# yinwoods/k8s-scheduler

Measured on AMD Instinct MI355X. Metric: pod-node evaluations/sec, higher is better.
Workload: dtype f64

## Files before the change

### include/ksched.h

```cpp
#ifndef KSCHED_H
#define KSCHED_H

#include <stddef.h>
#include <stdint.h>

#ifdef __cplusplus
extern "C" {
#endif

#define KSCHED_ABI_VERSION 6

#define KSCHED_OK 0
#define KSCHED_E_INVALID (-1)
#define KSCHED_E_DEVICE (-2)
#define KSCHED_E_PARSE (-3)
#define KSCHED_E_STATE (-4)
#define KSCHED_E_NOMEM (-5)
#define KSCHED_E_UNKNOWN_NODE (-6)

#define KSCHED_NO_FIT (-1)
#define KSCHED_NO_POSITIVE_SCORE (-2)
#define KSCHED_GANG_REJECTED (-3)

#define KSCHED_MODE_EXACT 0
// ... 158 lines not shown

int ksched_upload_pods(ksched_ctx *ctx, int64_t p, const int64_t *req_cpu, const int64_t *req_mem,
                       const int64_t *req_pods, const uint64_t *selector);
int ksched_run(ksched_ctx *ctx);
int ksched_set_timeout(ksched_ctx *ctx, int32_t persist_ms);
int ksched_sync(ksched_ctx *ctx);
int ksched_download_results(ksched_ctx *ctx, int64_t p, int32_t *out_idx, double *out_score, int32_t *out_feasible);
int ksched_get_stats(const ksched_ctx *ctx, ksched_stats *out);
int ksched_get_commit_stamps(const ksched_ctx *ctx, int32_t n, int64_t *out);
int ksched_get_seed_stats(const ksched_ctx *ctx, int64_t *out);
int ksched_set_timing(ksched_ctx *ctx, int32_t timing, int32_t every);

int ksched_selftest_fastdiv(ksched_ctx *ctx, int64_t n, const double *a, const double *b, double *out_native,
                            double *out_fast);
int ksched_selftest_score(ksched_ctx *ctx, int64_t n, const int64_t *req, const int64_t *alloc, double *out_score,
                          double *out_upper, double *out_recip, int32_t *out_flags);
int ksched_selftest_price_key(ksched_ctx *ctx, int64_t n, const float *price, double *out_key);
int ksched_selftest_screen(ksched_ctx *ctx, int64_t n, const int64_t *req, const int64_t *alloc, float *out_f32,
                           uint32_t *out_u32);
int ksched_selftest_rec_w(ksched_ctx *ctx, int64_t n, const float *w, const float *w2, uint32_t *out);
int ksched_selftest_threshold(ksched_ctx *ctx, int64_t n, const float *L, const uint32_t *rec, int32_t *out);
int ksched_selftest_seed(ksched_ctx *ctx, int64_t n, const float *v, const float *L, const uint32_t *flags,
                         const uint32_t *x, uint32_t *out);
int ksched_selftest_wave(ksched_ctx *ctx, int64_t ncases, const uint64_t *sort_code, const int32_t *sort_idx,
                         const double *key, const int32_t *idx, const int32_t *aux, const int32_t *cut,
                         const int32_t *nv, uint64_t *out_u64, int32_t *out_i32);
int ksched_selftest_list(ksched_ctx *ctx, int64_t n, int32_t steps, const double *key, const int32_t *idx,
                         double *out_key, int32_t *out_idx);
int ksched_selftest_slots(ksched_ctx *ctx, int64_t n, int32_t steps, const uint32_t *x, uint32_t *out);
int ksched_selftest_rank_merge(ksched_ctx *ctx, int32_t K, int32_t R, int32_t nb, const void *blocks, void *out_rec,
                               int64_t *out_fc);
int ksched_selftest_commit(ksched_ctx *ctx, int32_t impl, int32_t K, int32_t B, int32_t priority, int32_t domain,
                           int32_t use_labels, int32_t fast53, int32_t nb, const int64_t *rc, const int64_t *rm,
                           const int64_t *rp, const uint64_t *sel, const void *lists, const int64_t *fc0,
                           const void *xin, int32_t *out_idx, double *out_score, int32_t *out_feas, void *out_x,
                           int64_t *out_ctl);

int ksched_parse_cpu(const char *s, int64_t *out);
int ksched_parse_memory(const char *s, int64_t *out);
int ksched_parse_pods(const char *s, int64_t *out);
int ksched_parse_price(const char *s, float *out);

int ksched_pack_nodes(int64_t n, const char *const *names, const char *const *cap_cpu,
                      const char *const *cap_mem, const char *const *cap_pods,
                      int64_t nb, const char *const *bound_node, const int64_t *cont_off,
                      const char *const *cont_cpu, const char *const *cont_mem,
// ... 9 lines not shown
```

### k8s-scheduler_amd/csrc/ksched_commit.h

```cpp
#pragma once

#include <hip/hip_runtime.h>

#include <type_traits>

#ifndef KSCHED_XCHG_DEBUG
#define KSCHED_XCHG_DEBUG 0
#endif

#include "ksched_pipe.h"

namespace ksched {

namespace {

constexpr int kSpcHashBits = 11;
constexpr int kSpcHash = 1 << kSpcHashBits;
template <bool LAG3>
constexpr int spc_slots() { return LAG3 ? 192 : 128; }
static_assert(spc_slots<true>() + 1 <= kRescueMaxT, "RescueReq::ti must hold the persistent commit's touched slots");
constexpr int kSpcInvalid = kSpcHash - 1;
constexpr int kGS = 14;

constexpr uint64_t kSkipKeyBits = 0x7ff8000000000badull;
__device__ __forceinline__ double skip_key() { return __longlong_as_double((long long)kSkipKeyBits); }
__device__ __forceinline__ float screen_y(int64_t a, double y) {
    return (a > 0 && a < (1ll << 52)) ? (float)y : __builtin_nanf("");
}

struct alignas(8) SpcSlot {
    int32_t idx;
    int32_t mine;
    int64_t sb[3];
    int64_t cur[3];
    uint64_t labels;
    float price;
    int32_t pad;
};
static_assert(sizeof(SpcSlot) == 72, "SpcSlot");

struct SpcSmem {
    int32_t *hk;
    int64_t *s0;
    double *iy;
    int32_t *HP;
    uint32_t *tkc;
    int32_t *ti;
    SpcSlot *T;
    double *S;
    double *LK;
    int32_t *LI;
    int8_t *D;
    int32_t *fcg;
    int32_t *dfacc;
    int32_t *gn;
    int32_t *gq;
    int32_t *gs;
    double *pbk;
    int64_t *pbx;
    int32_t *ctl;
    int32_t *own;
    uint64_t *GS;
    float *thr;
    int16_t *x2s;
    float *rb2;
};

// ... 271 lines not shown
        m.pbk = reinterpret_cast<double *>(p); p += (size_t)kSpcWaves * 64 * sizeof(double);
        m.pbx = reinterpret_cast<int64_t *>(p); p += (size_t)kSpcWaves * 64 * sizeof(int64_t);
        m.LK = reinterpret_cast<double *>(p); p += (size_t)K * 64 * sizeof(double);
        m.GS = reinterpret_cast<uint64_t *>(p); p += 64 * kGS * sizeof(uint64_t);
        m.D = reinterpret_cast<int8_t *>(p); p += 64 * 64;
        m.T = reinterpret_cast<SpcSlot *>(p); p += (size_t)spc_slots<LAG3>() * sizeof(SpcSlot);
        m.LI = reinterpret_cast<int32_t *>(p); p += (size_t)K * 64 * sizeof(int32_t);
        m.HP = reinterpret_cast<int32_t *>(p); p += (size_t)K * 64 * sizeof(int32_t);
        m.hk = reinterpret_cast<int32_t *>(p); p += kSpcHash * sizeof(int32_t);
        m.tkc = reinterpret_cast<uint32_t *>(p); p += 64 * sizeof(uint32_t);
        m.ti = reinterpret_cast<int32_t *>(p); p += spc_slots<LAG3>() * sizeof(int32_t);
        m.fcg = reinterpret_cast<int32_t *>(p); p += 64 * sizeof(int32_t);
        m.dfacc = reinterpret_cast<int32_t *>(p); p += 64 * sizeof(int32_t);
        m.gn = reinterpret_cast<int32_t *>(p); p += 64 * sizeof(int32_t);
        m.gq = reinterpret_cast<int32_t *>(p); p += 64 * sizeof(int32_t);
        m.gs = reinterpret_cast<int32_t *>(p); p += 64 * sizeof(int32_t);
        m.ctl = reinterpret_cast<int32_t *>(p); p += 4 * sizeof(int32_t);
        m.thr = reinterpret_cast<float *>(p); p += 64 * sizeof(float);
        m.x2s = reinterpret_cast<int16_t *>(p); p += 64 * sizeof(int16_t);
        m.S = reinterpret_cast<double *>(p);
        m.own = reinterpret_cast<int32_t *>(m.pbk);
        m.s0 = reinterpret_cast<int64_t *>(m.D);
        m.iy = reinterpret_cast<double *>(m.GS);
        m.rb2 = reinterpret_cast<float *>(m.dfacc);
    }
    const int nb = (int)((A.pods.p - p0 < A.B) ? A.pods.p - p0 : A.B);
    const bool pj = lane < nb;
    const LanePods lp = pre ? *pre : load_lane_pods<LAB>(A.pods, p0, nb);
    const int64_t rc = lp.rc, rm = lp.rm, rp = lp.rp;
    const uint64_t sel = lp.sel;
    constexpr int kHeadPer = (64 * K + kSpcThreads - 1) / kSpcThreads;
    uint64_t w0[kHeadPer], w1[kHeadPer];
    int64_t fc0v = 0;
    int cut0 = 0;
    int32_t thr0 = 0;
    auto load_lists = [&]() {
        fc0v = (wave == 0 && pj) ? load_i64<COH>(A.fc0 + lane) : 0;
        cut0 = (wave == 0 && pj) ? (int32_t)(uint32_t)(load_i64<COH>(
                                       reinterpret_cast<const int64_t *>(A.lists + (size_t)lane * K) + 6) >> 32) : 0;
        if (SCR)
            thr0 = (wave == 0 && pj) ? (int32_t)(uint32_t)(load_i64<COH>(
                                           reinterpret_cast<const int64_t *>(A.lists + (size_t)lane * K + 1) + 6) >> 32) : 0;
#pragma unroll
        for (int u = 0; u < kHeadPer; ++u) {
            const int e = tid + u * kSpcThreads;
            w0[u] = 0; w1[u] = 0;
            if (e < 64 * K && e / K < nb) {
                const uint64_t *w = reinterpret_cast<const uint64_t *>(A.lists + e);
                if (COH) { w0[u] = ld_coh(w); w1[u] = ld_coh(w + 1); }
                else { w0[u] = w[0]; w1[u] = w[1]; }
            }
        }
    };
    if constexpr (!COH) load_lists();

    int n1 = 0, n2 = 0, nin = 0;
    uint64_t dbg_x1 = 0;
    (void)dbg_x1;
    const double rcf = (double)rc, rmf = (double)rm, rpf = (double)rp;
    const double y3 = recip(3.0);
    double *Srow = m.S + (size_t)lane * kSpcRow;
    uint64_t smv[3] = {0, 0, 0};
    auto key_inherited = [&](int ne, auto sl) {
        int dfl = 0;
        double pk = -__builtin_inf();
        int32_t pi = kNoIdx, ps = -1;
        const float thrf = SCR ? m.thr[lane] : 0.0f;
        const float qc = screen_req(rc), qm = screen_req(rm), qp = screen_req(rp);
        int64_t nex = 0;
        for (int e = wave; e < ne; e += kSpcWaves) {
            const int t = sl(e);
            const SpcSlot &x = m.T[t];
            const int64_t *x0 = m.s0 + e * 3;
            const bool f0 = fits(rc, rm, rp, sel, x0[0], x0[1], x0[2], x.labels, LAB);
            const bool f1 = fits(rc, rm, rp, sel, x.cur[0], x.cur[1], x.cur[2], x.labels, LAB);
            dfl += (int)f1 - (int)f0;
            const double *yy = m.iy + e * 6;
            bool need = true;
            if constexpr (SCR) {
                bool lo;
                const float v = screen_pair(qc, qm, qp, screen_y(x.cur[0], yy[3]), screen_y(x.cur[1], yy[4]),
                                            screen_y(x.cur[2], yy[5]), x.cur[0] >= rc, x.cur[1] >= rm, x.cur[2] >= rp, &lo);
                need = pj && !(v < thrf);
            }
            double k;
            if (!SCR || __ballot(need) != 0) {
                ++nex;
                const bool el = pair_key_fast<PRIO, DOM, F53>(f1, rc, rm, rp, rcf, rmf, rpf, x.cur[0], x.cur[1], x.cur[2],
                                                              yy[0], yy[1], yy[2], yy[3], yy[4], yy[5], y3, x.price, &k);
                k = el ? k : -__builtin_inf();
            } else {
                k = skip_key();
            }
            Srow[t] = k;
            const bool up = k != -__builtin_inf() && better(k, x.idx, pk, pi);
            pk = up ? k : pk; pi = up ? x.idx : pi; ps = up ? t : ps;
        }
        m.pbk[wave * 64 + lane] = pk;
        m.pbx[wave * 64 + lane] = ((int64_t)ps << 32) | (uint32_t)pi;
        if (dfl != 0) atomicAdd(&m.dfacc[lane], dfl);
        if (SCR && A.dbg && lane == 0 && wave < ne) {
            atomicAdd(reinterpret_cast<unsigned long long *>(&A.dbg[16]), (unsigned long long)((ne - 1 - wave) / kSpcWaves + 1));
            atomicAdd(reinterpret_cast<unsigned long long *>(&A.dbg[17]), (unsigned long long)nex);
        }
    };
    auto hash_lists = [&]() {
#pragma unroll
        for (int u = 0; u < kHeadPer; ++u) {
            const int e = tid + u * kSpcThreads;
            if (e < 64 * K) {
                const int j = e / K, q = e % K;
                const bool v = (uint32_t)(w1[u] >> 32) != 0;
                const double key = v ? __longlong_as_double((long long)w0[u]) : -__builtin_inf();
                const int32_t idx = v ? (int32_t)(uint32_t)w1[u] : kNoIdx;
                m.LK[q * 64 + j] = key;
                m.LI[q * 64 + j] = idx;
                m.HP[q * 64 + j] = idx == kNoIdx ? kSpcInvalid : spc_pos_insert(m.hk, idx);
// ... 132 lines not shown
        if (A.xp && A.xp->xdbg && wave == 0) {
            int64_t x = lane < n1 ? (int64_t)dbg_mix((uint64_t)xi.idx ^ ((uint64_t)xi.cur[0] << 20), (uint64_t)xi.cur[1] ^
                                                     (uint64_t)xi.cur[2] ^ (uint64_t)xi.sb[0], lane) : 0;
            x = wave_sum_i64(x);
            dbg_x1 = (uint64_t)x;
        }
#endif
        if (wave == 0) {
            int h = 0;
            bool dup = false;
            if (lane < n1) {
                h = spc_pos_insert(m.hk, xi.idx);
                dup = (m.tkc[h >> 5] >> (h & 31)) & 1u;
            }
            const uint64_t nm = __ballot(lane < n1 && !dup);
            const int slot = dup ? m.own[h] : n2 + __popcll(nm & ((1ull << lane) - 1ull));
            if (lane < n1) {
                SpcSlot &x = m.T[slot];
                x.idx = xi.idx; x.mine = 0;
                for (int r = 0; r < 3; ++r) { m.s0[lane * 3 + r] = xi.sb[r]; x.sb[r] = xi.cur[r]; x.cur[r] = xi.cur[r]; }
                x.labels = xi.labels; x.price = xi.price; x.pad = 0;
                m.ti[slot] = xi.idx;
                m.gs[lane] = slot;
                stage_state(m.iy + lane * 6, xi.cur);
                if (dup) m.x2s[slot] = -1;
                else atomicOr(&m.tkc[h >> 5], 1u << (h & 31));
            }
            if (lane == 0) m.ctl[3] = n2 + __popcll(nm);
        }
        __syncthreads();
        if (tid == 0 && A.trace_row) A.trace_row[23] = wall_clock64();
        nin = m.ctl[3];
        key_inherited(n1, [&](int e) { return (int)m.gs[e]; });
        __syncthreads();
        if (tid == 0 && A.trace_row) A.trace_row[24] = wall_clock64();
    }

    int32_t fcc = 0;
    double rbk = -__builtin_inf();
    int32_t rbi = kNoIdx, rbs = -1;
    constexpr bool RB2 = COH && PRIO == kPrioResource && DOM == kDomAll;
    bool trk = false;
    int cv = 0, cut = 0;
    int32_t my_idx = 0, my_feas = 0;
    int32_t my_src = 0;
    double my_score = 0.0;
    int32_t my_g = -2, my_q = -1, my_s = -1, my_h = kSpcInvalid;
// ... 158 lines not shown
            const bool in = lane >= c && lane < cend;
            if (in && my_g == 0) my_g = m.LI[my_q * 64 + lane];
            m.gn[lane] = in ? my_g : -2;
            m.gq[lane] = my_q;
            m.gs[lane] = my_s;
            m.fcg[lane] = 0;
            if (lane == 0) { m.ctl[0] = c; m.ctl[1] = cend; }
        }
        __syncthreads();
        if (first && tr1) tr1[49] = wall_clock64();
        if (dbg) { const uint64_t t = __builtin_amdgcn_s_memtime(); t_s1 += t - t_mark; t_mark = t; }
        const int rc0 = m.ctl[0], rce = m.ctl[1];
        {
            double pk = -__builtin_inf();
            int32_t pi = kNoIdx, ps = -1;
            if (wave == 0 && lane >= rc0 && lane < rce && m.gn[lane] >= 0) {
                const uint64_t *src = reinterpret_cast<const uint64_t *>(A.lists + (size_t)lane * K + m.gq[lane]) + 2;
                uint64_t v[5];
#pragma unroll
                for (int w = 0; w < 5; ++w) v[w] = COH ? ld_coh(src + w) : src[w];
                const int64_t n0 = wsub((int64_t)v[0], rc), n1 = wsub((int64_t)v[1], rm), n2 = wsub((int64_t)v[2], 1);
                const double nf0 = (double)n0, nf1 = (double)n1, nf2 = (double)n2;
                uint64_t *o = m.GS + (size_t)lane * kGS;
#pragma unroll
                for (int w = 0; w < 5; ++w) o[w] = v[w];
                o[5] = (uint64_t)n0; o[6] = (uint64_t)n1; o[7] = (uint64_t)n2;
                o[8] = (uint64_t)__double_as_longlong(nf0); o[9] = (uint64_t)__double_as_longlong(nf1);
                o[10] = (uint64_t)__double_as_longlong(nf2);
                o[11] = (uint64_t)__double_as_longlong(recip_or_zero(n0, nf0));
                o[12] = (uint64_t)__double_as_longlong(recip_or_zero(n1, nf1));
                o[13] = (uint64_t)__double_as_longlong(recip_or_zero(n2, nf2));
            }
            __syncthreads();
            const float thrf = SCR ? m.thr[lane] : 0.0f;
            const float qc = screen_req(rc), qm = screen_req(rm), qp = screen_req(rp);
            int64_t nev = 0, nex = 0;
            for (int k = rc0 + wave; k < rce; k += kSpcWaves) {
                const int32_t g = __builtin_amdgcn_readfirstlane(m.gn[k]);
                if (g < 0) continue;
                const int s = __builtin_amdgcn_readfirstlane(m.gs[k]);
                const uint64_t *gsk = m.GS + (size_t)k * kGS;
                const int64_t a0 = (int64_t)gsk[0], a1 = (int64_t)gsk[1], a2 = (int64_t)gsk[2];
                const uint64_t lab = gsk[3];
                const float pr = __uint_as_float((uint32_t)gsk[4]);
                const int64_t n0 = (int64_t)gsk[5], n1 = (int64_t)gsk[6], n2 = (int64_t)gsk[7];
                const bool fo = fits(rc, rm, rp, sel, a0, a1, a2, lab, LAB);
                const bool fn = fits(rc, rm, rp, sel, n0, n1, n2, lab, LAB);
                const int d = (int)fn - (int)fo;
                const double ny0 = __longlong_as_double((long long)gsk[11]), ny1 = __longlong_as_double((long long)gsk[12]),
                             ny2 = __longlong_as_double((long long)gsk[13]);
                bool need = true;
                if constexpr (SCR) {
                    bool lo;
                    const float v = screen_pair(qc, qm, qp, screen_y(n0, ny0), screen_y(n1, ny1), screen_y(n2, ny2),
                                                n0 >= rc, n1 >= rm, n2 >= rp, &lo);
                    need = lane > k && pj && !(v < thrf);
                }
                double kv;
                ++nev;
                if (!SCR || __ballot(need) != 0) {
                    ++nex;
                    const bool el = pair_key_fast<PRIO, DOM, F53>(
                        fn, rc, rm, rp, rcf, rmf, rpf, n0, n1, n2, __longlong_as_double((long long)gsk[8]),
                        __longlong_as_double((long long)gsk[9]), __longlong_as_double((long long)gsk[10]), ny0, ny1, ny2,
                        y3, pr, &kv);
                    kv = el ? kv : -__builtin_inf();
                } else {
                    kv = skip_key();
                }
                Srow[s] = kv;
                m.D[k * 64 + lane] = (int8_t)d;
                if (lane > k) {
                    if (d != 0) atomicAdd(&m.fcg[lane], d);
                    const bool up = kv != -__builtin_inf() && better(kv, g, pk, pi);
                    pk = up ? kv : pk; pi = up ? g : pi; ps = up ? s : ps;
                }
                if (lane == 0) {
                    SpcSlot &x = m.T[s];
                    x.idx = g; x.mine = 1;
                    x.sb[0] = a0; x.sb[1] = a1; x.sb[2] = a2;
                    x.cur[0] = n0; x.cur[1] = n1; x.cur[2] = n2;
                    x.labels = lab; x.price = pr; x.pad = 0;
                    m.ti[s] = g;
                }
            }
            m.pbk[wave * 64 + lane] = pk;
            m.pbx[wave * 64 + lane] = ((int64_t)ps << 32) | (uint32_t)pi;
            if (SCR && A.dbg && lane == 0 && nev) {
                atomicAdd(reinterpret_cast<unsigned long long *>(&A.dbg[18]), (unsigned long long)nev);
                atomicAdd(reinterpret_cast<unsigned long long *>(&A.dbg[19]), (unsigned long long)nex);
            }
        }
        __syncthreads();
        if (first && tr1) tr1[50] = wall_clock64();
        if (dbg) { const uint64_t t = __builtin_amdgcn_s_memtime(); t_s2 += t - t_mark; t_mark = t; }
        if (wave == 0) {
            ++nrounds;
            const int cend = rce;
            double tk = rbk;
            int32_t ti = rbi, ts = rbs;
            for (int w = 0; w < kSpcWaves; ++w) {
                const double k = m.pbk[w * 64 + lane];
                const int64_t x = m.pbx[w * 64 + lane];
                const int32_t xi = (int32_t)(uint32_t)x;
                const bool up = k != -__builtin_inf() && better(k, xi, tk, ti);
                tk = up ? k : tk; ti = up ? xi : ti; ts = up ? (int32_t)(x >> 32) : ts;
// ... 145 lines not shown
                    if (kf != 0) {
                        ++placed;
                        int64_t b0, b1, b2;
                        uint64_t lab;
                        float pr;
                        if (kf == 1 && rescued) {
                            b0 = ro.a[0]; b1 = ro.a[1]; b2 = ro.a[2]; lab = ro.labels; pr = ro.price;
                            s = nT++;
                        } else if (kf == 1) {
                            int64_t ra[3];
                            load_rec_state<COH>(A.lists + (size_t)f * K + qf, ra, &lab, &pr);
                            b0 = ra[0]; b1 = ra[1]; b2 = ra[2];
                            s = nT++;
                        } else {
                            const SpcSlot &x = m.T[s];
                            b0 = x.cur[0]; b1 = x.cur[1]; b2 = x.cur[2]; lab = x.labels; pr = x.price;
                        }
                        const int64_t n0 = wsub(b0, rl64(rc, f)), n1 = wsub(b1, rl64(rm, f)), n2 = wsub(b2, 1);
                        const bool fo = fits(rc, rm, rp, sel, b0, b1, b2, lab, LAB);
                        const bool fn = fits(rc, rm, rp, sel, n0, n1, n2, lab, LAB);
                        fcc += (int32_t)fn - (int32_t)fo;
                        double kv;
                        if constexpr (SCR) {
                            const double nf0 = (double)n0, nf1 = (double)n1, nf2 = (double)n2;
                            const double ny0 = recip_or_zero(n0, nf0), ny1 = recip_or_zero(n1, nf1),
                                         ny2 = recip_or_zero(n2, nf2);
                            bool lo;
                            const float v = screen_pair(screen_req(rc), screen_req(rm), screen_req(rp), screen_y(n0, ny0),
                                                        screen_y(n1, ny1), screen_y(n2, ny2), n0 >= rc, n1 >= rm, n2 >= rp,
                                                        &lo);
                            const bool need = lane > f && pj && !(v < m.thr[lane]);
                            const bool any = __ballot(need) != 0;
                            if (any) {
                                const bool el = pair_key_fast<PRIO, DOM, F53>(fn, rc, rm, rp, rcf, rmf, rpf, n0, n1, n2, nf0,
                                                                              nf1, nf2, ny0, ny1, ny2, y3, pr, &kv);
                                kv = el ? kv : -__builtin_inf();
                            } else {
                                kv = skip_key();
                            }
                            if (A.dbg && lane == 0) {
                                atomicAdd(reinterpret_cast<unsigned long long *>(&A.dbg[20]), 1ull);
                                if (any) atomicAdd(reinterpret_cast<unsigned long long *>(&A.dbg[21]), 1ull);
                            }
                        } else {
                            kv = lane_key<PRIO, DOM, LAB, F53>(fn, rc, rm, rp, rcf, rmf, rpf, n0, n1, n2, y3, pr);
                        }
                        Srow[s] = kv;
                        if (lane == 0) {
                            SpcSlot &x = m.T[s];
                            if (kf == 1) {
                                x.idx = wi;
                                x.sb[0] = b0; x.sb[1] = b1; x.sb[2] = b2;
                                x.labels = lab; x.price = pr; x.pad = 0;
                                m.ti[s] = wi;
                                const int pos = rescued ? spc_pos_insert(m.hk, wi) : m.HP[qf * 64 + f];
                                m.tkc[pos >> 5] |= 1u << (pos & 31);
                            }
                            x.mine = 1;
                            x.cur[0] = n0; x.cur[1] = n1; x.cur[2] = n2;
                        }
                        lds_order();
                        const bool up = kv != -__builtin_inf() && better(kv, wi, rbk, rbi);
// ... 161 lines not shown
            if (done < nb) __hip_atomic_fetch_add(st + 1, 1ull, __ATOMIC_RELAXED, __HIP_MEMORY_SCOPE_AGENT);
            __hip_atomic_fetch_add(st + 2, (unsigned long long)placed, __ATOMIC_RELAXED, __HIP_MEMORY_SCOPE_AGENT);
            if (nresc) __hip_atomic_fetch_add(st + 4, (unsigned long long)nresc, __ATOMIC_RELAXED, __HIP_MEMORY_SCOPE_AGENT);
        }
        if (threadIdx.x == 0) A.loc->rescue_credit = rcredit - 4 * nresc;
    }
    return 1;
}

template <int K, int NT = kSpcThreads, bool LAG3 = false>
constexpr size_t spc_small_bytes() {
    return (size_t)(NT / 64) * 64 * 16 + (size_t)K * 64 * 8 + 64 * kGS * 8 + 64 * 64 + spc_slots<LAG3>() * sizeof(SpcSlot) +
           (size_t)K * 64 * 8 + (size_t)kSpcHash * 4 + 64 * 4 + spc_slots<LAG3>() * 4 + 5 * 64 * 4 + 16 + 64 * 4 + 64 * 2;
}
template <int K, int NT = kSpcThreads, bool LAG3 = false>
constexpr size_t spc_lds_bytes() {
    return (size_t)64 * (spc_slots<LAG3>() + 1) * 8 + (size_t)(NT / 64) * 64 * 16 + (size_t)K * 64 * 12 +
           spc_slots<LAG3>() * sizeof(SpcSlot) + (size_t)kSpcHash * 4 + (size_t)K * 64 * 4 + 64 * 4 +
           spc_slots<LAG3>() * 4 + 5 * 64 * 4 + 16 + 64 * kGS * 8 + 64 * 4 + 64 * 2 + 64 * 64;
}
static_assert(spc_lds_bytes<16>() <= 160 * 1024, "k_commit_spc LDS");
static_assert(spc_lds_bytes<16, kPipeThreads, true>() == spc_small_bytes<16, kPipeThreads, true>() + 64 * 193 * 8,
              "SpcSmem: S last");
static_assert(64 * 64 >= 128 * 3 * 8 && 64 * kGS * 8 >= 128 * 6 * 8, "SpcSmem prologue aliases");
static_assert((size_t)(kSpcThreads / 64) * 64 * 16 >= kSpcHash * 4 && (kPipeThreads / 64) * 64 * 16 >= kSpcHash * 4,
              "SpcSmem::own aliases pbk/pbx");

}
```

### k8s-scheduler_amd/csrc/ksched_data.hip

```cpp
#include <cmath>
#include <cstring>

#include <new>

#include "ksched_ctx.h"
#include "ksched_preempt.h"
#include "ksched_rank.h"

using namespace ksched;

static uint64_t uabs(int64_t v) { return v < 0 ? (uint64_t)0 - (uint64_t)v : (uint64_t)v; }

bool ksched::build_bound_table(int64_t n, int64_t nb, const int32_t *node_idx, const int64_t *cpu, const int64_t *mem,
                               const int32_t *prio, BoundTableHost *out, const char **why) {
    const int64_t blocks = (n + 63) / 64;
    out->seg.assign((size_t)n, 0);
    for (int64_t t = 0; t < nb; ++t) {
        if (node_idx[t] < 0 || node_idx[t] >= n) { *why = "node index out of range"; return false; }
        if (++out->seg[(size_t)node_idx[t]] > kBoundMaxPerNode) { *why = "more than KSCHED_BOUND_MAX_PER_NODE pods on one node"; return false; }
    }
    std::vector<int64_t> start((size_t)n + 1, 0);
    for (int64_t j = 0; j < n; ++j) start[(size_t)j + 1] = start[(size_t)j] + out->seg[(size_t)j];
    std::vector<int32_t> order((size_t)nb);
    {
// ... 375 lines not shown

int ksched_selftest_threshold(ksched_ctx *c, int64_t n, const float *L, const uint32_t *rec, int32_t *out) {
    if (!c || n < 0 || (n > 0 && (!L || !rec || !out))) return KSCHED_E_INVALID;
    if (n == 0) return KSCHED_OK;
    const size_t q = (size_t)n;
    return selftest_run(c, "selftest_threshold", {{L, nullptr, q * 4}, {rec, nullptr, q * 4}, {nullptr, out, q * 16}},
                        [&](const std::vector<void *> &p) {
                            return launch_selftest_threshold(n, (const float *)p[0], (const uint32_t *)p[1],
                                                             (int32_t *)p[2], c->stream);
                        });
}

int ksched_selftest_seed(ksched_ctx *c, int64_t n, const float *v, const float *L, const uint32_t *flags,
                         const uint32_t *x, uint32_t *out) {
    if (!c || n < 0 || (n > 0 && (!v || !L || !flags || !x || !out))) return KSCHED_E_INVALID;
    if (n == 0) return KSCHED_OK;
    const size_t q = (size_t)n;
    return selftest_run(c, "selftest_seed",
                        {{v, nullptr, q * 4}, {L, nullptr, q * 4}, {flags, nullptr, q * 4}, {x, nullptr, q * 24},
                         {nullptr, out, q * 20}},
                        [&](const std::vector<void *> &p) {
                            return launch_selftest_seed(n, (const float *)p[0], (const float *)p[1], (const uint32_t *)p[2],
                                                        (const uint32_t *)p[3], (uint32_t *)p[4], c->stream);
                        });
}

int ksched_selftest_wave(ksched_ctx *c, int64_t ncases, const uint64_t *sort_code, const int32_t *sort_idx,
                         const double *key, const int32_t *idx, const int32_t *aux, const int32_t *cut,
                         const int32_t *nv, uint64_t *out_u64, int32_t *out_i32) {
    if (!c || ncases < 0 || ncases > (1 << 20) ||
        (ncases > 0 && (!sort_code || !sort_idx || !key || !idx || !aux || !cut || !nv || !out_u64 || !out_i32)))
        return KSCHED_E_INVALID;
    if (ncases == 0) return KSCHED_OK;
    const size_t l = (size_t)ncases * 64;
    return selftest_run(c, "selftest_wave",
                        {{sort_code, nullptr, l * 6 * 8}, {sort_idx, nullptr, l * 6 * 4}, {key, nullptr, l * 8},
                         {idx, nullptr, l * 4}, {aux, nullptr, l * 4}, {cut, nullptr, (size_t)ncases * 4},
                         {nv, nullptr, (size_t)ncases * 4}, {nullptr, out_u64, l * 12 * 8}, {nullptr, out_i32, l * 13 * 4}},
                        [&](const std::vector<void *> &p) {
                            WaveTestArgs a{};
                            a.ncases = ncases;
                            a.scode = (const uint64_t *)p[0]; a.sidx = (const int32_t *)p[1];
                            a.key = (const double *)p[2]; a.kidx = (const int32_t *)p[3]; a.aux = (const int32_t *)p[4];
                            a.cut = (const int32_t *)p[5]; a.nv = (const int32_t *)p[6];
                            uint64_t *u = (uint64_t *)p[7];
                            int32_t *v = (int32_t *)p[8];
// ... 302 lines not shown
```

### k8s-scheduler_amd/csrc/ksched_kernels.h

```cpp
#pragma once

#include "ksched_device.h"

namespace ksched {

struct alignas(16) XRec {
    int32_t idx;
    int32_t pad;
    int64_t cur[3];
    int64_t sb[3];
    uint64_t labels;
    float price;
    int32_t pad2;
    int64_t pad3;
};
static_assert(sizeof(XRec) == 80, "XRec layout");

template <bool COH>
__device__ __forceinline__ void add_i64(int64_t *p, int64_t v) {
    if (COH) st_coh(p, (uint64_t)((int64_t)ld_coh(p) + v)); else *p += v;
}

struct alignas(16) XBuf {
    int32_t count;
// ... 165 lines not shown
    const int32_t *kidx, *aux;
    const int32_t *cut, *nv;
    uint64_t *ocode;
    int32_t *oidx;
    int32_t *rank;
    uint64_t *red_max;
    int64_t *red_sum;
    int32_t *red_min;
    uint64_t *red_or;
    uint64_t *ab_key;
    int32_t *ab_idx, *ab_aux;
    uint64_t *kcode;
    int32_t *thr;
};
hipError_t launch_selftest_score(int64_t n, const int64_t *req, const int64_t *alloc, double *score, double *upper,
                                 double *rcp, int32_t *flags, hipStream_t s);
hipError_t launch_selftest_price(int64_t n, const float *price, double *key, hipStream_t s);
hipError_t launch_selftest_screen(int64_t n, const int64_t *req, const int64_t *alloc, float *f, uint32_t *u,
                                  hipStream_t s);
hipError_t launch_selftest_rec_w(int64_t n, const float *w, const float *w2, uint32_t *out, hipStream_t s);
hipError_t launch_selftest_threshold(int64_t n, const float *L, const uint32_t *rec, int32_t *out, hipStream_t s);
hipError_t launch_selftest_seed(int64_t n, const float *v, const float *L, const uint32_t *flags, const uint32_t *x,
                                uint32_t *out, hipStream_t s);
hipError_t launch_selftest_wave(const WaveTestArgs &a, hipStream_t s);
hipError_t launch_selftest_list(int64_t n, int S, const double *key, const int32_t *idx, double *okey, int32_t *oidx,
                                hipStream_t s);
hipError_t launch_selftest_slots(int64_t n, int steps, const uint32_t *x, uint32_t *out, hipStream_t s);

#define KSCHED_DISPATCH(prio, dom, lab, f53, CALL)                                              \
    do {                                                                                        \
        if ((prio) == kPrioPrice) {                                                             \
            constexpr int P_ = kPrioPrice, D_ = kDomFeasible; constexpr bool F_ = false;        \
            if (lab) { constexpr bool L_ = true; return CALL; }                                 \
            else { constexpr bool L_ = false; return CALL; }                                    \
        }                                                                                       \
        constexpr int P_ = kPrioResource;                                                       \
        if ((dom) == kDomFeasible) {                                                            \
            constexpr int D_ = kDomFeasible;                                                    \
            if (lab) { constexpr bool L_ = true;                                                \
                if (f53) { constexpr bool F_ = true; return CALL; } else { constexpr bool F_ = false; return CALL; } } \
            else { constexpr bool L_ = false;                                                   \
                if (f53) { constexpr bool F_ = true; return CALL; } else { constexpr bool F_ = false; return CALL; } } \
        } else {                                                                                \
            constexpr int D_ = kDomAll;                                                         \
            if (lab) { constexpr bool L_ = true;                                                \
                if (f53) { constexpr bool F_ = true; return CALL; } else { constexpr bool F_ = false; return CALL; } } \
// ... 7 lines not shown
```

### k8s-scheduler_amd/csrc/ksched_selftest.hip

```cpp
#include <hip/hip_runtime.h>

#include <cstring>

#include "ksched_commit.h"
#include "ksched_ctx.h"
#include "ksched_merge.h"
#include "ksched_stream.h"

namespace ksched {

namespace {

struct PairOps {
    int64_t r[3], a[3];
    double rf[3], af[3], y[3], y3;
};
__device__ __forceinline__ PairOps load_ops(int64_t n, int64_t i, const int64_t *req, const int64_t *alloc) {
    PairOps o;
#pragma unroll
    for (int k = 0; k < 3; ++k) {
        o.r[k] = req[k * n + i];
        o.a[k] = alloc[k * n + i];
        o.rf[k] = (double)o.r[k];
        o.af[k] = (double)o.a[k];
// ... 92 lines not shown
    out[2 * n + i] = pk & 0xffffu;
    out[3 * n + i] = pk >> 16;
}

__global__ void k_selftest_threshold(int64_t n, const float *L, const uint32_t *rec, int32_t *out) {
    const int64_t i = (int64_t)blockIdx.x * blockDim.x + threadIdx.x;
    if (i >= n) return;
    const int tq = screen_rec_threshold(L[i]), tqn = screen_rec_threshold_nf(L[i]);
    out[i] = tq;
    out[n + i] = tqn;
    out[2 * n + i] = screen_rec_needed(rec[i], tq, tqn) ? 1 : 0;
    out[3 * n + i] = screen_rec_needed(rec[i], -1, -1) ? 1 : 0;
}

__global__ void k_selftest_seed(int64_t n, const float *v, const float *L, const uint32_t *flags, const uint32_t *x,
                                uint32_t *out) {
    const int64_t i = (int64_t)blockIdx.x * blockDim.x + threadIdx.x;
    if (i >= n) return;
    out[i] = screen_need(v[i], (flags[i] & 1u) != 0, (flags[i] & 2u) != 0, L[i]) ? 1u : 0u;
    uint32_t t[4] = {0u, 0u, 0u, 0u};
    for (int s = 0; s < 6; ++s) bound_insert<4>(t, x[s * n + i]);
#pragma unroll
    for (int q = 0; q < 4; ++q) out[(1 + q) * n + i] = t[q];
}

template <int RUN>
__device__ __forceinline__ void sort_case(const WaveTestArgs &A, int r, int64_t nl, int64_t i, int lane) {
    uint64_t c = A.scode[r * nl + i];
    int32_t x = A.sidx[r * nl + i];
    wave_sort_desc<RUN>(c, x, lane);
    A.ocode[r * nl + i] = c;
    A.oidx[r * nl + i] = x;
}

__global__ __launch_bounds__(64) void k_selftest_wave(WaveTestArgs A) {
    const int64_t cs = blockIdx.x;
    if (cs >= A.ncases || threadIdx.x >= 64) return;
    const int lane = (int)threadIdx.x;
    const int64_t nl = A.ncases * 64, i = cs * 64 + lane;
    sort_case<1>(A, 0, nl, i, lane);
    sort_case<2>(A, 1, nl, i, lane);
    sort_case<4>(A, 2, nl, i, lane);
    sort_case<8>(A, 3, nl, i, lane);
    sort_case<16>(A, 4, nl, i, lane);
    sort_case<32>(A, 5, nl, i, lane);
    const uint64_t c0 = A.scode[i];
// ... 79 lines not shown
}

namespace {
dim3 grid_of(int64_t n) { return dim3((unsigned)((n + 255) / 256)); }
}

hipError_t launch_selftest_score(int64_t n, const int64_t *req, const int64_t *alloc, double *score, double *upper,
                                 double *rcp, int32_t *flags, hipStream_t s) {
    if (n <= 0) return hipSuccess;
    hipLaunchKernelGGL(k_selftest_score, grid_of(n), dim3(256), 0, s, n, req, alloc, score, upper, rcp, flags);
    return hipGetLastError();
}

hipError_t launch_selftest_price(int64_t n, const float *price, double *key, hipStream_t s) {
    if (n <= 0) return hipSuccess;
    hipLaunchKernelGGL(k_selftest_price, grid_of(n), dim3(256), 0, s, n, price, key);
    return hipGetLastError();
}

hipError_t launch_selftest_screen(int64_t n, const int64_t *req, const int64_t *alloc, float *f, uint32_t *u,
                                  hipStream_t s) {
    if (n <= 0) return hipSuccess;
    hipLaunchKernelGGL(k_selftest_screen, grid_of(n), dim3(256), 0, s, n, req, alloc, f, u);
    return hipGetLastError();
}

hipError_t launch_selftest_rec_w(int64_t n, const float *w, const float *w2, uint32_t *out, hipStream_t s) {
    if (n <= 0) return hipSuccess;
    hipLaunchKernelGGL(k_selftest_rec_w, grid_of(n), dim3(256), 0, s, n, w, w2, out);
    return hipGetLastError();
}

hipError_t launch_selftest_seed(int64_t n, const float *v, const float *L, const uint32_t *flags, const uint32_t *x,
                                uint32_t *out, hipStream_t s) {
    if (n <= 0) return hipSuccess;
    hipLaunchKernelGGL(k_selftest_seed, grid_of(n), dim3(256), 0, s, n, v, L, flags, x, out);
    return hipGetLastError();
}

hipError_t launch_selftest_threshold(int64_t n, const float *L, const uint32_t *rec, int32_t *out, hipStream_t s) {
    if (n <= 0) return hipSuccess;
    hipLaunchKernelGGL(k_selftest_threshold, grid_of(n), dim3(256), 0, s, n, L, rec, out);
    return hipGetLastError();
}

hipError_t launch_selftest_wave(const WaveTestArgs &a, hipStream_t s) {
// ... 146 lines not shown
```

### k8s-scheduler_amd/ksched/_lib.py

```python
from __future__ import annotations

import ctypes as C
import os

PKG_ROOT = os.path.dirname(os.path.dirname(os.path.abspath(__file__)))
LIB_PATH = os.environ.get("KSCHED_LIB") or os.path.join(PKG_ROOT, "libksched.so")
HEADER_PATH = os.path.join(os.path.dirname(PKG_ROOT), "include", "ksched.h")

OK = 0
E_INVALID = -1
E_DEVICE = -2
E_PARSE = -3
E_STATE = -4
E_NOMEM = -5
E_UNKNOWN_NODE = -6
NO_FIT = -1
NO_POSITIVE_SCORE = -2
GANG_REJECTED = -3

ABI_VERSION = 6
XCHG_RINGS_UNCACHED, XCHG_RINGS_IPC = 1, 2
MODE_EXACT, MODE_BATCHED, MODE_AUTO = 0, 1, 2
PIPELINE_AUTO, PIPELINE_STREAM = 0, 1
PRIORITY_RESOURCE, PRIORITY_BEST_PRICE = 0, 1
# ... 87 lines not shown
    ("ksched_read_spread", C.c_int, [CTX, I32P]),
    ("ksched_schedule_spread", C.c_int, [CTX, C.c_int64, I64P, I64P, I64P, U64P, I32P, U8P, I32P, F64P, I32P]),
    ("ksched_load_ext", C.c_int, [CTX, C.c_int32, I64P]),
    ("ksched_read_ext", C.c_int, [CTX, I64P]),
    ("ksched_schedule_ext", C.c_int, [CTX, C.c_int64, I64P, I64P, I64P, U64P, I64P, I32P, F64P, I32P]),
    ("ksched_schedule_constrained", C.c_int, [CTX, C.c_int64, I64P, I64P, I64P, U64P, C.c_int64, I64P, I32P, I32P, U8P,
                                              I64P, I32P, F64P, I32P, I32P]),
    ("ksched_upload_pods", C.c_int, [CTX, C.c_int64, I64P, I64P, I64P, U64P]),
    ("ksched_run", C.c_int, [CTX]),
    ("ksched_sync", C.c_int, [CTX]),
    ("ksched_download_results", C.c_int, [CTX, C.c_int64, I32P, F64P, I32P]),
    ("ksched_get_stats", C.c_int, [CTX, C.POINTER(Stats)]),
    ("ksched_get_commit_stamps", C.c_int, [CTX, C.c_int32, I64P]),
    ("ksched_get_seed_stats", C.c_int, [CTX, I64P]),
    ("ksched_set_timing", C.c_int, [CTX, C.c_int32, C.c_int32]),
    ("ksched_set_timeout", C.c_int, [CTX, C.c_int32]),
    ("ksched_selftest_fastdiv", C.c_int, [CTX, C.c_int64, F64P, F64P, F64P, F64P]),
    ("ksched_selftest_score", C.c_int, [CTX, C.c_int64, I64P, I64P, F64P, F64P, F64P, I32P]),
    ("ksched_selftest_price_key", C.c_int, [CTX, C.c_int64, F32P, F64P]),
    ("ksched_selftest_screen", C.c_int, [CTX, C.c_int64, I64P, I64P, F32P, U32P]),
    ("ksched_selftest_rec_w", C.c_int, [CTX, C.c_int64, F32P, F32P, U32P]),
    ("ksched_selftest_threshold", C.c_int, [CTX, C.c_int64, F32P, U32P, I32P]),
    ("ksched_selftest_seed", C.c_int, [CTX, C.c_int64, F32P, F32P, U32P, U32P, U32P]),
    ("ksched_selftest_wave", C.c_int, [CTX, C.c_int64, U64P, I32P, F64P, I32P, I32P, I32P, I32P, U64P, I32P]),
    ("ksched_selftest_list", C.c_int, [CTX, C.c_int64, C.c_int32, F64P, I32P, F64P, I32P]),
    ("ksched_selftest_slots", C.c_int, [CTX, C.c_int64, C.c_int32, U32P, U32P]),
    ("ksched_selftest_rank_merge", C.c_int, [CTX, C.c_int32, C.c_int32, C.c_int32, C.c_void_p, C.c_void_p, I64P]),
    ("ksched_selftest_commit", C.c_int, [CTX] + [C.c_int32] * 8 + [I64P, I64P, I64P, U64P, C.c_void_p, I64P, C.c_void_p,
                                         I32P, F64P, I32P, C.c_void_p, I64P]),
    ("ksched_parse_cpu", C.c_int, [C.c_char_p, I64P]),
    ("ksched_parse_memory", C.c_int, [C.c_char_p, I64P]),
    ("ksched_parse_pods", C.c_int, [C.c_char_p, I64P]),
    ("ksched_parse_price", C.c_int, [C.c_char_p, F32P]),
    ("ksched_pack_nodes", C.c_int, [C.c_int64, STRV, STRV, STRV, STRV, C.c_int64, STRV, I64P, STRV, STRV,
                                    I64P, I64P, I64P]),
    ("ksched_pack_pods", C.c_int, [C.c_int64, I64P, STRV, STRV, I64P, I64P, I64P]),
]


def lib():
    global _lib
    if _lib is None:
        if not os.path.exists(LIB_PATH):
            raise ImportError(f"{LIB_PATH} not built: run `make -C {PKG_ROOT}` (no CPU fallback exists)")
        lb = C.CDLL(LIB_PATH)
        ab = bool(os.environ.get("KSCHED_LIB"))
# ... 24 lines not shown
```

Before: 290.6 billion.

## Stage touched-node screen floats in LDS and preload slot indices per wave

In the screened commit path, the float screen values (TouchY) for each touched slot are precomputed once when the slot state is staged, instead of being rebuilt from doubles per pod lane. The slot table writes now happen in the staging lane rather than lane 0 inside the loop. Slot indices are loaded once per wave into a register and read back with readlane, avoiding a serialized LDS read each iteration. The screen-plus-key logic moves into a shared touch_column helper, and a new selftest covers it. The cost is extra LDS aliasing inside GS and a more complex staging phase.

```diff
diff --git a/include/ksched.h b/include/ksched.h
--- a/include/ksched.h
+++ b/include/ksched.h
@@ -204,6 +204,8 @@
 int ksched_selftest_threshold(ksched_ctx *ctx, int64_t n, const float *L, const uint32_t *rec, int32_t *out);
 int ksched_selftest_seed(ksched_ctx *ctx, int64_t n, const float *v, const float *L, const uint32_t *flags,
                          const uint32_t *x, uint32_t *out);
+int ksched_selftest_touch_screen(ksched_ctx *ctx, int64_t n, const int64_t *req, const int64_t *alloc, const float *thr,
+                                 const uint32_t *active, float *out_f32, uint32_t *out_u32, double *out_key);
 int ksched_selftest_wave(ksched_ctx *ctx, int64_t ncases, const uint64_t *sort_code, const int32_t *sort_idx,
                          const double *key, const int32_t *idx, const int32_t *aux, const int32_t *cut,
                          const int32_t *nv, uint64_t *out_u64, int32_t *out_i32);
diff --git a/k8s-scheduler_amd/csrc/ksched_commit.h b/k8s-scheduler_amd/csrc/ksched_commit.h
--- a/k8s-scheduler_amd/csrc/ksched_commit.h
+++ b/k8s-scheduler_amd/csrc/ksched_commit.h
@@ -26,6 +26,36 @@
 __device__ __forceinline__ double skip_key() { return __longlong_as_double((long long)kSkipKeyBits); }
 __device__ __forceinline__ float screen_y(int64_t a, double y) {
     return (a > 0 && a < (1ll << 52)) ? (float)y : __builtin_nanf("");
+}
+
+struct alignas(16) TouchY {
+    float c, m, p, w;
+};
+__device__ __forceinline__ TouchY touch_stage(int64_t a0, int64_t a1, int64_t a2, double y0, double y1, double y2) {
+    return TouchY{screen_y(a0, y0), screen_y(a1, y1), screen_y(a2, y2), 0.0f};
+}
+__device__ __forceinline__ bool touch_need(float qc, float qm, float qp, float thr, const TouchY &ty, int64_t rc, int64_t rm,
+                                           int64_t rp, int64_t n0, int64_t n1, int64_t n2, bool active, float *v) {
+    bool lo;
+    *v = screen_pair(qc, qm, qp, ty.c, ty.m, ty.p, n0 >= rc, n1 >= rm, n2 >= rp, &lo);
+    return active && !(*v < thr);
+}
+template <int PRIO, int DOM, bool F53>
+__device__ __forceinline__ bool touch_column(float qc, float qm, float qp, float thr, const TouchY &ty, bool active,
+                                             bool feas, int64_t rc, int64_t rm, int64_t rp, double rcf, double rmf,
+                                             double rpf, int64_t n0, int64_t n1, int64_t n2, const double *fy, double y3,
+                                             float pr, double *key) {
+    float v;
+    const bool need = touch_need(qc, qm, qp, thr, ty, rc, rm, rp, n0, n1, n2, active, &v);
+    if (__ballot(need) == 0) {
+        *key = skip_key();
+        return false;
+    }
+    double k;
+    const bool el = pair_key_fast<PRIO, DOM, F53>(feas, rc, rm, rp, rcf, rmf, rpf, n0, n1, n2, fy[0], fy[1], fy[2], fy[3],
+                                                  fy[4], fy[5], y3, pr, &k);
+    *key = el ? k : -__builtin_inf();
+    return true;
 }
 
 struct alignas(8) SpcSlot {
@@ -43,6 +73,7 @@
     int32_t *hk;
     int64_t *s0;
     double *iy;
+    TouchY *iyt;
     int32_t *HP;
     uint32_t *tkc;
     int32_t *ti;
@@ -360,6 +391,7 @@
         m.own = reinterpret_cast<int32_t *>(m.pbk);
         m.s0 = reinterpret_cast<int64_t *>(m.D);
         m.iy = reinterpret_cast<double *>(m.GS);
+        m.iyt = reinterpret_cast<TouchY *>(m.iy + 128 * 6);
         m.rb2 = reinterpret_cast<float *>(m.dfacc);
     }
     const int nb = (int)((A.pods.p - p0 < A.B) ? A.pods.p - p0 : A.B);
@@ -406,31 +438,33 @@
         const float thrf = SCR ? m.thr[lane] : 0.0f;
         const float qc = screen_req(rc), qm = screen_req(rm), qp = screen_req(rp);
         int64_t nex = 0;
-        for (int e = wave; e < ne; e += kSpcWaves) {
-            const int t = sl(e);
+        int tv = 0;
+        if constexpr (SCR) {
+            const int ev = wave + lane * kSpcWaves;
+            tv = ev < ne ? sl(ev) : 0;
+        }
+        for (int e = wave, u = 0; e < ne; e += kSpcWaves, ++u) {
+            const int t = SCR ? __builtin_amdgcn_readlane(tv, u) : sl(e);
             const SpcSlot &x = m.T[t];
             const int64_t *x0 = m.s0 + e * 3;
             const bool f0 = fits(rc, rm, rp, sel, x0[0], x0[1], x0[2], x.labels, LAB);
             const bool f1 = fits(rc, rm, rp, sel, x.cur[0], x.cur[1], x.cur[2], x.labels, LAB);
             dfl += (int)f1 - (int)f0;
             const double *yy = m.iy + e * 6;
-            bool need = true;
+            double k;
             if constexpr (SCR) {
-                bool lo;
-                const float v = screen_pair(qc, qm, qp, screen_y(x.cur[0], yy[3]), screen_y(x.cur[1], yy[4]),
-                                            screen_y(x.cur[2], yy[5]), x.cur[0] >= rc, x.cur[1] >= rm, x.cur[2] >= rp, &lo);
-                need = pj && !(v < thrf);
-            }
-            double k;
-            if (!SCR || __ballot(need) != 0) {
+                const bool any = touch_column<PRIO, DOM, F53>(qc, qm, qp, thrf, m.iyt[e], pj, f1, rc, rm, rp, rcf, rmf, rpf,
+                                                              x.cur[0], x.cur[1], x.cur[2], yy, y3, x.price, &k);
+                Srow[t] = k;
+                if (!any) continue;
+                ++nex;
+            } else {
                 ++nex;
                 const bool el = pair_key_fast<PRIO, DOM, F53>(f1, rc, rm, rp, rcf, rmf, rpf, x.cur[0], x.cur[1], x.cur[2],
                                                               yy[0], yy[1], yy[2], yy[3], yy[4], yy[5], y3, x.price, &k);
                 k = el ? k : -__builtin_inf();
-            } else {
-                k = skip_key();
-            }
-            Srow[t] = k;
+                Srow[t] = k;
+            }
             const bool up = k != -__builtin_inf() && better(k, x.idx, pk, pi);
             pk = up ? k : pk; pi = up ? x.idx : pi; ps = up ? t : ps;
         }
@@ -609,7 +643,15 @@
                 x.labels = xi.labels; x.price = xi.price; x.pad = 0;
                 m.ti[slot] = xi.idx;
                 m.gs[lane] = slot;
-                stage_state(m.iy + lane * 6, xi.cur);
+                if constexpr (SCR) {
+                    double st[6];
+                    stage_state(st, xi.cur);
+#pragma unroll
+                    for (int r = 0; r < 6; ++r) m.iy[lane * 6 + r] = st[r];
+                    m.iyt[lane] = touch_stage(xi.cur[0], xi.cur[1], xi.cur[2], st[3], st[4], st[5]);
+                } else {
+                    stage_state(m.iy + lane * 6, xi.cur);
+                }
                 if (dup) m.x2s[slot] = -1;
                 else atomicOr(&m.tkc[h >> 5], 1u << (h & 31));
             }
@@ -814,66 +856,102 @@
                 const int64_t n0 = wsub((int64_t)v[0], rc), n1 = wsub((int64_t)v[1], rm), n2 = wsub((int64_t)v[2], 1);
                 const double nf0 = (double)n0, nf1 = (double)n1, nf2 = (double)n2;
                 uint64_t *o = m.GS + (size_t)lane * kGS;
-#pragma unroll
-                for (int w = 0; w < 5; ++w) o[w] = v[w];
-                o[5] = (uint64_t)n0; o[6] = (uint64_t)n1; o[7] = (uint64_t)n2;
-                o[8] = (uint64_t)__double_as_longlong(nf0); o[9] = (uint64_t)__double_as_longlong(nf1);
-                o[10] = (uint64_t)__double_as_longlong(nf2);
-                o[11] = (uint64_t)__double_as_longlong(recip_or_zero(n0, nf0));
-                o[12] = (uint64_t)__double_as_longlong(recip_or_zero(n1, nf1));
-                o[13] = (uint64_t)__double_as_longlong(recip_or_zero(n2, nf2));
+                if constexpr (SCR) {
+                    const double ny0 = recip_or_zero(n0, nf0), ny1 = recip_or_zero(n1, nf1), ny2 = recip_or_zero(n2, nf2);
+                    SpcSlot &x = m.T[my_s];
+                    x.idx = my_g; x.mine = 1;
+                    x.sb[0] = (int64_t)v[0]; x.sb[1] = (int64_t)v[1]; x.sb[2] = (int64_t)v[2];
+                    x.cur[0] = n0; x.cur[1] = n1; x.cur[2] = n2;
+                    x.labels = v[3]; x.price = __uint_as_float((uint32_t)v[4]); x.pad = 0;
+                    m.ti[my_s] = my_g;
+                    *reinterpret_cast<TouchY *>(o) = touch_stage(n0, n1, n2, ny0, ny1, ny2);
+                    o[8] = (uint64_t)__double_as_longlong(nf0); o[9] = (uint64_t)__double_as_longlong(nf1);
+                    o[10] = (uint64_t)__double_as_longlong(nf2);
+                    o[11] = (uint64_t)__double_as_longlong(ny0);
+                    o[12] = (uint64_t)__double_as_longlong(ny1);
+                    o[13] = (uint64_t)__double_as_longlong(ny2);
+                } else {
+#pragma unroll
+                    for (int w = 0; w < 5; ++w) o[w] = v[w];
+                    o[5] = (uint64_t)n0; o[6] = (uint64_t)n1; o[7] = (uint64_t)n2;
+                    o[8] = (uint64_t)__double_as_longlong(nf0); o[9] = (uint64_t)__double_as_longlong(nf1);
+                    o[10] = (uint64_t)__double_as_longlong(nf2);
+                    o[11] = (uint64_t)__double_as_longlong(recip_or_zero(n0, nf0));
+                    o[12] = (uint64_t)__double_as_longlong(recip_or_zero(n1, nf1));
+                    o[13] = (uint64_t)__double_as_longlong(recip_or_zero(n2, nf2));
+                }
             }
             __syncthreads();
             const float thrf = SCR ? m.thr[lane] : 0.0f;
             const float qc = screen_req(rc), qm = screen_req(rm), qp = screen_req(rp);
             int64_t nev = 0, nex = 0;
-            for (int k = rc0 + wave; k < rce; k += kSpcWaves) {
-                const int32_t g = __builtin_amdgcn_readfirstlane(m.gn[k]);
-                if (g < 0) continue;
-                const int s = __builtin_amdgcn_readfirstlane(m.gs[k]);
-                const uint64_t *gsk = m.GS + (size_t)k * kGS;
-                const int64_t a0 = (int64_t)gsk[0], a1 = (int64_t)gsk[1], a2 = (int64_t)gsk[2];
-                const uint64_t lab = gsk[3];
-                const float pr = __uint_as_float((uint32_t)gsk[4]);
-                const int64_t n0 = (int64_t)gsk[5], n1 = (int64_t)gsk[6], n2 = (int64_t)gsk[7];
-                const bool fo = fits(rc, rm, rp, sel, a0, a1, a2, lab, LAB);
-                const bool fn = fits(rc, rm, rp, sel, n0, n1, n2, lab, LAB);
-                const int d = (int)fn - (int)fo;
-                const double ny0 = __longlong_as_double((long long)gsk[11]), ny1 = __longlong_as_double((long long)gsk[12]),
-                             ny2 = __longlong_as_double((long long)gsk[13]);
-                bool need = true;
+            int32_t sv = -1;
+            if constexpr (SCR) {
+                const int kk = rc0 + wave + lane * kSpcWaves;
+                if (kk < rce) sv = m.gs[kk];
+            }
+            for (int k = rc0 + wave, u = 0; k < rce; k += kSpcWaves, ++u) {
                 if constexpr (SCR) {
-                    bool lo;
-                    const float v = screen_pair(qc, qm, qp, screen_y(n0, ny0), screen_y(n1, ny1), screen_y(n2, ny2),
-                                                n0 >= rc, n1 >= rm, n2 >= rp, &lo);
-                    need = lane > k && pj && !(v < thrf);
-                }
-                double kv;
-                ++nev;
-                if (!SCR || __ballot(need) != 0) {
+                    const int s = __builtin_amdgcn_readlane(sv, u);
+                    if (s < 0) continue;
+                    const SpcSlot &x = m.T[s];
+                    const uint64_t *gsk = m.GS + (size_t)k * kGS;
+                    const int64_t n0 = x.cur[0], n1 = x.cur[1], n2 = x.cur[2];
+                    const bool fo = fits(rc, rm, rp, sel, x.sb[0], x.sb[1], x.sb[2], x.labels, LAB);
+                    const bool fn = fits(rc, rm, rp, sel, n0, n1, n2, x.labels, LAB);
+                    const int d = (int)fn - (int)fo;
+                    double kv;
+                    ++nev;
+                    const bool any = touch_column<PRIO, DOM, F53>(
+                        qc, qm, qp, thrf, *reinterpret_cast<const TouchY *>(gsk), lane > k && pj, fn, rc, rm, rp, rcf, rmf,
+                        rpf, n0, n1, n2, reinterpret_cast<const double *>(gsk + 8), y3, x.price, &kv);
+                    Srow[s] = kv;
+                    m.D[k * 64 + lane] = (int8_t)d;
+                    if (lane > k && d != 0) atomicAdd(&m.fcg[lane], d);
+                    if (!any) continue;
+                    ++nex;
+                    if (lane > k) {
+                        const int32_t g = x.idx;
+                        const bool up = kv != -__builtin_inf() && better(kv, g, pk, pi);
+                        pk = up ? kv : pk; pi = up ? g : pi; ps = up ? s : ps;
+                    }
+                } else {
+                    const int32_t g = __builtin_amdgcn_readfirstlane(m.gn[k]);
+                    if (g < 0) continue;
+                    const int s = __builtin_amdgcn_readfirstlane(m.gs[k]);
+                    const uint64_t *gsk = m.GS + (size_t)k * kGS;
+                    const int64_t a0 = (int64_t)gsk[0], a1 = (int64_t)gsk[1], a2 = (int64_t)gsk[2];
+                    const uint64_t lab = gsk[3];
+                    const float pr = __uint_as_float((uint32_t)gsk[4]);
+                    const int64_t n0 = (int64_t)gsk[5], n1 = (int64_t)gsk[6], n2 = (int64_t)gsk[7];
+                    const bool fo = fits(rc, rm, rp, sel, a0, a1, a2, lab, LAB);
+                    const bool fn = fits(rc, rm, rp, sel, n0, n1, n2, lab, LAB);
+                    const int d = (int)fn - (int)fo;
+                    const double ny0 = __longlong_as_double((long long)gsk[11]), ny1 = __longlong_as_double((long long)gsk[12]),
+                                 ny2 = __longlong_as_double((long long)gsk[13]);
+                    double kv;
+                    ++nev;
                     ++nex;
                     const bool el = pair_key_fast<PRIO, DOM, F53>(
                         fn, rc, rm, rp, rcf, rmf, rpf, n0, n1, n2, __longlong_as_double((long long)gsk[8]),
                         __longlong_as_double((long long)gsk[9]), __longlong_as_double((long long)gsk[10]), ny0, ny1, ny2,
                         y3, pr, &kv);
                     kv = el ? kv : -__builtin_inf();
-                } else {
-                    kv = skip_key();
-                }
-                Srow[s] = kv;
-                m.D[k * 64 + lane] = (int8_t)d;
-                if (lane > k) {
-                    if (d != 0) atomicAdd(&m.fcg[lane], d);
-                    const bool up = kv != -__builtin_inf() && better(kv, g, pk, pi);
-                    pk = up ? kv : pk; pi = up ? g : pi; ps = up ? s : ps;
-                }
-                if (lane == 0) {
-                    SpcSlot &x = m.T[s];
-                    x.idx = g; x.mine = 1;
-                    x.sb[0] = a0; x.sb[1] = a1; x.sb[2] = a2;
-                    x.cur[0] = n0; x.cur[1] = n1; x.cur[2] = n2;
-                    x.labels = lab; x.price = pr; x.pad = 0;
-                    m.ti[s] = g;
+                    Srow[s] = kv;
+                    m.D[k * 64 + lane] = (int8_t)d;
+                    if (lane > k) {
+                        if (d != 0) atomicAdd(&m.fcg[lane], d);
+                        const bool up = kv != -__builtin_inf() && better(kv, g, pk, pi);
+                        pk = up ? kv : pk; pi = up ? g : pi; ps = up ? s : ps;
+                    }
+                    if (lane == 0) {
+                        SpcSlot &x = m.T[s];
+                        x.idx = g; x.mine = 1;
+                        x.sb[0] = a0; x.sb[1] = a1; x.sb[2] = a2;
+                        x.cur[0] = n0; x.cur[1] = n1; x.cur[2] = n2;
+                        x.labels = lab; x.price = pr; x.pad = 0;
+                        m.ti[s] = g;
+                    }
                 }
             }
             m.pbk[wave * 64 + lane] = pk;
@@ -1065,22 +1143,13 @@
                         fcc += (int32_t)fn - (int32_t)fo;
                         double kv;
                         if constexpr (SCR) {
-                            const double nf0 = (double)n0, nf1 = (double)n1, nf2 = (double)n2;
-                            const double ny0 = recip_or_zero(n0, nf0), ny1 = recip_or_zero(n1, nf1),
-                                         ny2 = recip_or_zero(n2, nf2);
-                            bool lo;
-                            const float v = screen_pair(screen_req(rc), screen_req(rm), screen_req(rp), screen_y(n0, ny0),
-                                                        screen_y(n1, ny1), screen_y(n2, ny2), n0 >= rc, n1 >= rm, n2 >= rp,
-                                                        &lo);
-                            const bool need = lane > f && pj && !(v < m.thr[lane]);
-                            const bool any = __ballot(need) != 0;
-                            if (any) {
-                                const bool el = pair_key_fast<PRIO, DOM, F53>(fn, rc, rm, rp, rcf, rmf, rpf, n0, n1, n2, nf0,
-                                                                              nf1, nf2, ny0, ny1, ny2, y3, pr, &kv);
-                                kv = el ? kv : -__builtin_inf();
-                            } else {
-                                kv = skip_key();
-                            }
+                            const int64_t nn[3] = {n0, n1, n2};
+                            double st[6];
+                            stage_state(st, nn);
+                            const bool any = touch_column<PRIO, DOM, F53>(
+                                screen_req(rc), screen_req(rm), screen_req(rp), m.thr[lane],
+                                touch_stage(n0, n1, n2, st[3], st[4], st[5]), lane > f && pj, fn, rc, rm, rp, rcf, rmf, rpf,
+                                n0, n1, n2, st, y3, pr, &kv);
                             if (A.dbg && lane == 0) {
                                 atomicAdd(reinterpret_cast<unsigned long long *>(&A.dbg[20]), 1ull);
                                 if (any) atomicAdd(reinterpret_cast<unsigned long long *>(&A.dbg[21]), 1ull);
@@ -1288,7 +1357,8 @@
 static_assert(spc_lds_bytes<16>() <= 160 * 1024, "k_commit_spc LDS");
 static_assert(spc_lds_bytes<16, kPipeThreads, true>() == spc_small_bytes<16, kPipeThreads, true>() + 64 * 193 * 8,
               "SpcSmem: S last");
-static_assert(64 * 64 >= 128 * 3 * 8 && 64 * kGS * 8 >= 128 * 6 * 8, "SpcSmem prologue aliases");
+static_assert(64 * 64 >= 128 * 3 * 8 && 64 * kGS * 8 >= 128 * 6 * 8 + 64 * sizeof(TouchY), "SpcSmem prologue aliases");
+static_assert(sizeof(TouchY) == 16 && kGS * 8 % 16 == 0 && kGS >= 14, "SpcSmem::GS rows hold a TouchY");
 static_assert((size_t)(kSpcThreads / 64) * 64 * 16 >= kSpcHash * 4 && (kPipeThreads / 64) * 64 * 16 >= kSpcHash * 4,
               "SpcSmem::own aliases pbk/pbx");
 
diff --git a/k8s-scheduler_amd/csrc/ksched_data.hip b/k8s-scheduler_amd/csrc/ksched_data.hip
--- a/k8s-scheduler_amd/csrc/ksched_data.hip
+++ b/k8s-scheduler_amd/csrc/ksched_data.hip
@@ -421,6 +421,22 @@
                         [&](const std::vector<void *> &p) {
                             return launch_selftest_seed(n, (const float *)p[0], (const float *)p[1], (const uint32_t *)p[2],
                                                         (const uint32_t *)p[3], (uint32_t *)p[4], c->stream);
+                        });
+}
+
+int ksched_selftest_touch_screen(ksched_ctx *c, int64_t n, const int64_t *req, const int64_t *alloc, const float *thr,
+                                 const uint32_t *active, float *out_f32, uint32_t *out_u32, double *out_key) {
+    if (!c || n < 0 || (n > 0 && (!req || !alloc || !thr || !active || !out_f32 || !out_u32 || !out_key)))
+        return KSCHED_E_INVALID;
+    if (n == 0) return KSCHED_OK;
+    const size_t q = (size_t)n;
+    return selftest_run(c, "selftest_touch_screen",
+                        {{req, nullptr, q * 24}, {alloc, nullptr, q * 24}, {thr, nullptr, q * 4}, {active, nullptr, q * 4},
+                         {nullptr, out_f32, q * 16}, {nullptr, out_u32, q * 8}, {nullptr, out_key, q * 8}},
+                        [&](const std::vector<void *> &p) {
+                            return launch_selftest_touch_screen(n, (const int64_t *)p[0], (const int64_t *)p[1],
+                                                                (const float *)p[2], (const uint32_t *)p[3], (float *)p[4],
+                                                                (uint32_t *)p[5], (double *)p[6], c->stream);
                         });
 }
 
diff --git a/k8s-scheduler_amd/csrc/ksched_kernels.h b/k8s-scheduler_amd/csrc/ksched_kernels.h
--- a/k8s-scheduler_amd/csrc/ksched_kernels.h
+++ b/k8s-scheduler_amd/csrc/ksched_kernels.h
@@ -211,6 +211,8 @@
 hipError_t launch_selftest_threshold(int64_t n, const float *L, const uint32_t *rec, int32_t *out, hipStream_t s);
 hipError_t launch_selftest_seed(int64_t n, const float *v, const float *L, const uint32_t *flags, const uint32_t *x,
                                 uint32_t *out, hipStream_t s);
+hipError_t launch_selftest_touch_screen(int64_t n, const int64_t *req, const int64_t *alloc, const float *thr,
+                                        const uint32_t *active, float *f, uint32_t *u, double *key, hipStream_t s);
 hipError_t launch_selftest_wave(const WaveTestArgs &a, hipStream_t s);
 hipError_t launch_selftest_list(int64_t n, int S, const double *key, const int32_t *idx, double *okey, int32_t *oidx,
                                 hipStream_t s);
diff --git a/k8s-scheduler_amd/csrc/ksched_selftest.hip b/k8s-scheduler_amd/csrc/ksched_selftest.hip
--- a/k8s-scheduler_amd/csrc/ksched_selftest.hip
+++ b/k8s-scheduler_amd/csrc/ksched_selftest.hip
@@ -138,6 +138,30 @@
     for (int s = 0; s < 6; ++s) bound_insert<4>(t, x[s * n + i]);
 #pragma unroll
     for (int q = 0; q < 4; ++q) out[(1 + q) * n + i] = t[q];
+}
+
+__global__ void k_selftest_touch_screen(int64_t n, const int64_t *req, const int64_t *alloc, const float *thr,
+                                        const uint32_t *active, float *f, uint32_t *u, double *key) {
+    const int64_t i = (int64_t)blockIdx.x * blockDim.x + threadIdx.x;
+    const bool in = i < n;
+    const PairOps o = load_ops(n, in ? i : 0, req, alloc);
+    const TouchY ty = touch_stage(o.a[0], o.a[1], o.a[2], o.y[0], o.y[1], o.y[2]);
+    const float q0 = screen_req(o.r[0]), q1 = screen_req(o.r[1]), q2 = screen_req(o.r[2]);
+    const float th = in ? thr[i] : 0.0f;
+    const bool act = in && active[i] != 0;
+    float v;
+    const bool need = touch_need(q0, q1, q2, th, ty, o.r[0], o.r[1], o.r[2], o.a[0], o.a[1], o.a[2], act, &v);
+    const bool feas = fits(o.r[0], o.r[1], o.r[2], 0ull, o.a[0], o.a[1], o.a[2], 0ull, false);
+    const double fy[6] = {o.af[0], o.af[1], o.af[2], o.y[0], o.y[1], o.y[2]};
+    double k;
+    const bool any = touch_column<kPrioResource, kDomAll, false>(q0, q1, q2, th, ty, act, feas, o.r[0], o.r[1], o.r[2],
+                                                                 o.rf[0], o.rf[1], o.rf[2], o.a[0], o.a[1], o.a[2], fy, o.y3,
+                                                                 0.0f, &k);
+    if (!in) return;
+    f[i] = ty.c; f[n + i] = ty.m; f[2 * n + i] = ty.p; f[3 * n + i] = v;
+    u[i] = need ? 1u : 0u;
+    u[n + i] = any ? 1u : 0u;
+    key[i] = k;
 }
 
 template <int RUN>
@@ -263,6 +287,13 @@
                                   hipStream_t s) {
     if (n <= 0) return hipSuccess;
     hipLaunchKernelGGL(k_selftest_screen, grid_of(n), dim3(256), 0, s, n, req, alloc, f, u);
+    return hipGetLastError();
+}
+
+hipError_t launch_selftest_touch_screen(int64_t n, const int64_t *req, const int64_t *alloc, const float *thr,
+                                        const uint32_t *active, float *f, uint32_t *u, double *key, hipStream_t s) {
+    if (n <= 0) return hipSuccess;
+    hipLaunchKernelGGL(k_selftest_touch_screen, grid_of(n), dim3(256), 0, s, n, req, alloc, thr, active, f, u, key);
     return hipGetLastError();
 }
 
diff --git a/k8s-scheduler_amd/ksched/_lib.py b/k8s-scheduler_amd/ksched/_lib.py
--- a/k8s-scheduler_amd/ksched/_lib.py
+++ b/k8s-scheduler_amd/ksched/_lib.py
@@ -133,6 +133,7 @@
     ("ksched_selftest_rec_w", C.c_int, [CTX, C.c_int64, F32P, F32P, U32P]),
     ("ksched_selftest_threshold", C.c_int, [CTX, C.c_int64, F32P, U32P, I32P]),
     ("ksched_selftest_seed", C.c_int, [CTX, C.c_int64, F32P, F32P, U32P, U32P, U32P]),
+    ("ksched_selftest_touch_screen", C.c_int, [CTX, C.c_int64, I64P, I64P, F32P, U32P, F32P, U32P, F64P]),
     ("ksched_selftest_wave", C.c_int, [CTX, C.c_int64, U64P, I32P, F64P, I32P, I32P, I32P, I32P, U64P, I32P]),
     ("ksched_selftest_list", C.c_int, [CTX, C.c_int64, C.c_int32, F64P, I32P, F64P, I32P]),
     ("ksched_selftest_slots", C.c_int, [CTX, C.c_int64, C.c_int32, U32P, U32P]),
```

Result: faster. 300.7 billion (median of 6 runs) (+3.5%).
